# PRBonn/SHINE_mapping

Measured on NVIDIA H100. Metric: sdf_train_points_per_sec_fwd_bwd, higher is better.
Workload: dtype f32

## Files before the change

shine_mapping_b200/csrc/shine_b200.cu:

```cuda

#include <cuda_runtime.h>
#include <math.h>
#include <stdint.h>

#include <type_traits>

#include "shine_b200.h"

#ifndef SHINE_GATHER_GROUP
#define SHINE_GATHER_GROUP 2
#endif
#ifndef SHINE_TRAIN_MINB
#define SHINE_TRAIN_MINB 2
#endif
#ifndef SHINE_TRAIN_DECGRAD_MINB
#define SHINE_TRAIN_DECGRAD_MINB 1
#endif
#ifndef SHINE_INFER_MINB
#define SHINE_INFER_MINB 3
#endif

#include "shine_device.cuh"

namespace {


__global__ void hash_insert_kernel(HashSlot* __restrict__ slots, uint32_t mask, const int64_t* __restrict__ keys,
                                   const int32_t* __restrict__ corner_ids, int64_t n, int32_t node_base,
                                   int32_t* __restrict__ overflow) {
    const int64_t i = (int64_t)blockIdx.x * blockDim.x + threadIdx.x;
    if (i >= n) return;
// ... 214 lines not shown
}

__device__ __forceinline__ void to_afrag(const float (&v)[4], int odd, float (&a)[4]) {
    const float s0 = odd ? v[0] : v[2], s1 = odd ? v[1] : v[3];
    const float r0 = __shfl_xor_sync(kFull, s0, 1), r1 = __shfl_xor_sync(kFull, s1, 1);
    if (!odd) { a[0] = v[0]; a[2] = v[1]; a[1] = r0; a[3] = r1; }
    else      { a[0] = r0;   a[2] = r1;   a[1] = v[2]; a[3] = v[3]; }
}
__device__ __forceinline__ void from_cfrag(const float (&c)[4], int odd, float (&v)[4]) {
    const float s0 = odd ? c[0] : c[2], s1 = odd ? c[1] : c[3];
    const float r0 = __shfl_xor_sync(kFull, s0, 1), r1 = __shfl_xor_sync(kFull, s1, 1);
    if (!odd) { v[0] = c[0]; v[1] = c[1]; v[2] = r0; v[3] = r1; }
    else      { v[0] = r0;   v[1] = r1;   v[2] = c[2]; v[3] = c[3]; }
}

#define SHINE_ACC_DECL float dW2[2][4][4], dW1[2][4], db2p[4][2], db1p[4][2], dw3p[4][2]

__device__ __forceinline__ float reduce_scatter_g8(const float (&v)[8], int lane) {
    float a[4], b[2];
    const bool b4 = (lane & 16) != 0, b3 = (lane & 8) != 0, b2 = (lane & 4) != 0;
#pragma unroll
    for (int i = 0; i < 4; ++i) a[i] = (b4 ? v[4 + i] : v[i]) + __shfl_xor_sync(kFull, b4 ? v[i] : v[4 + i], 16);
#pragma unroll
    for (int i = 0; i < 2; ++i) b[i] = (b3 ? a[2 + i] : a[i]) + __shfl_xor_sync(kFull, b3 ? a[i] : a[2 + i], 8);
    return (b2 ? b[1] : b[0]) + __shfl_xor_sync(kFull, b2 ? b[0] : b[1], 4);
}

__device__ __forceinline__ int frag_chunk(int lane) { return lane ^ ((lane >> 2) & 6); }
template <int NTF>
__device__ __forceinline__ void load_afrag(const float* blk, int c, AFrag<NTF>& a) {
    const float4 v = *reinterpret_cast<const float4*>(blk + 4 * c);
    a.set_packed(v.x, v.y, v.z, v.w);
}
__device__ __forceinline__ void load_bfrag(const float* blk, int c, uint2& bh, uint2& bl) {
    const float2 v = *reinterpret_cast<const float2*>(blk + 2 * c);
    split_fast2(v.x, v.y, bh.x, bh.y, bl.x, bl.y);
}
__device__ __forceinline__ void stage_afrags(float* blk, const int (&sq)[2], const float (&c)[4][4]) {
#pragma unroll
    for (int mt = 0; mt < 2; ++mt)
#pragma unroll
        for (int q = 0; q < 2; ++q)
            *reinterpret_cast<float4*>(blk + 128 * mt + 4 * sq[q]) = make_float4(c[2 * mt][q], c[2 * mt + 1][q], c[2 * mt][2 + q], c[2 * mt + 1][2 + q]);
}
__device__ __forceinline__ int xfrag_word(int ks, int c) { return 64 * ks + 2 * (c ^ (8 * ks)); }
__device__ __forceinline__ void load_xfrag(const float* sx, int ks, int c, uint2& bh, uint2& bl) {
    const float2 v = *reinterpret_cast<const float2*>(sx + xfrag_word(ks, c));
    split_fast2(v.x, v.y, bh.x, bh.y, bl.x, bl.y);
}


constexpr int kGatherGroup = SHINE_GATHER_GROUP;

using shine_internal::StepParams;

struct SmemPlan {
    static constexpr int W1 = 0;
    static constexpr int W1T = W1 + 2 * kH * kF;
    static constexpr int W2 = W1T + 2 * kF * kWS;
    static constexpr int W3W2T = W2 + 2 * kH * kWS;
    static constexpr int B1 = W3W2T + 2 * kH * kWS;
    static constexpr int B2 = B1 + kH;
    static constexpr int W3 = B2 + kH;
    static constexpr int B3 = W3 + kH;
    static constexpr int GSCALE = B3 + 1;
    static constexpr int kDecGradFloats = kH * kF + kH + kH * kH + kH + kH + 1;
    static constexpr int ZSUM = B3 + 4;
    static constexpr int kZsumFloats = 8 * 5 * kTile;
    static constexpr int STAGE = ZSUM + kZsumFloats;
    static constexpr int SB2 = 0;
    static constexpr int SU = SB2;
    static constexpr int SA1 = SB2 + kTile * kH;
    static constexpr int SX = SA1 + kTile * kH;
    static constexpr int SA2 = SX + kTile * kF;
    static constexpr int SDP = SA2;
    static constexpr int kStagePerWarp = SA2 + kTile * kH;
    static constexpr int kStageGrouped = SDP + 2 * kTile;
    __host__ __device__ static constexpr int stage_per_warp(bool grouped) { return grouped ? kStageGrouped : kStagePerWarp; }
    static constexpr int kGroupPerLevel = 4 * kTile;
    static constexpr int kW2Part = kH * kH;
};

constexpr int kMaxGroupedRuns = 6;

__device__ __forceinline__ void red_add_f2(float* p, float a, float b) {
    asm volatile("red.global.add.v2.f32 [%0], {%1,%2};" ::"l"(p), "f"(a), "f"(b) : "memory");
}
__device__ __forceinline__ int group_slot(int p) { return 4 * (p & 3) + (p >> 2); }

template <int LMAX>
__device__ __forceinline__ void grouped_scatter(const StepParams& P, int L, int tile, const float* __restrict__ pt,
                                                float* __restrict__ dtile, const float (&dxc)[4], int lane) {
    const int g = lane >> 2, t = lane & 3;
    *reinterpret_cast<float2*>(dtile + g * kF + 2 * t) = make_float2(dxc[0], dxc[1]);
    *reinterpret_cast<float2*>(dtile + (g + 8) * kF + 2 * t) = make_float2(dxc[2], dxc[3]);
// ... 97 lines not shown
    shine_internal::BrickGrid g;
    __device__ __forceinline__ void load(const StepParams&, int64_t p, float& x, float& y, float& z) const {
        const int n1 = g.n + 1, per = n1 * n1 * n1;
        const int64_t b = p / per;
        const int r = (int)(p - b * per);
        const int i = r / (n1 * n1), j = (r / n1) % n1, k = r % n1;
        x = __fadd_rn(g.origin[0], __fmul_rn(g.spacing, (float)(__ldg(g.bricks + 3 * b) * g.n + i)));
        y = __fadd_rn(g.origin[1], __fmul_rn(g.spacing, (float)(__ldg(g.bricks + 3 * b + 1) * g.n + j)));
        z = __fadd_rn(g.origin[2], __fmul_rn(g.spacing, (float)(__ldg(g.bricks + 3 * b + 2) * g.n + k)));
    }
    __device__ __forceinline__ float out(float v) const { return -v; }
};

template <class Src>
constexpr int infer_min_blocks() { return std::is_same<Src, BatchCoords>::value ? SHINE_INFER_MINB : 2; }

template <int NTF, bool TRAIN, bool DEC_GRAD, int LMAX, bool GROUPED = false, class Src = BatchCoords>
__global__ void __launch_bounds__(256, !TRAIN ? infer_min_blocks<Src>() : (DEC_GRAD && !GROUPED) ? SHINE_TRAIN_DECGRAD_MINB : SHINE_TRAIN_MINB)
sdf_fused_kernel(const __grid_constant__ StepParams P, const __grid_constant__ Src src) {
    static_assert(std::is_same<Src, BatchCoords>::value || !TRAIN, "generated coordinates are for inference only");
    static_assert(!GROUPED || TRAIN, "the grouped scatter belongs to the training kernels");
    static_assert(!DEC_GRAD || TRAIN, "decoder gradients belong to the training kernels");
    static_assert(SmemPlan::kStagePerWarp >= SmemPlan::kDecGradFloats, "a warp's staging area holds its partial decoder gradient");
    static_assert(SmemPlan::kStageGrouped >= kH * kF + 3 * kH + 1, "a grouped warp's staging area holds its partial bias / dW1 gradients");
    static_assert(!(GROUPED && DEC_GRAD) ||
                      (SmemPlan::STAGE + 8 * (SmemPlan::kStageGrouped + LMAX * SmemPlan::kGroupPerLevel + SmemPlan::kW2Part)) * 4 + 1024 <=
                          227 * 1024 / SHINE_TRAIN_MINB,
                  "the grouped kernel's shared memory fits SHINE_TRAIN_MINB blocks/SM");
    extern __shared__ __align__(16) float smem[];
    uint32_t* smu = reinterpret_cast<uint32_t*>(smem);
    const int tid = threadIdx.x, lane = tid & 31, warp = tid >> 5;
    const int g = lane >> 2, t = lane & 3, odd = t & 1, half = t >> 1;
    constexpr int kWarps = 8;

    for (int i = tid; i < kH * kF; i += blockDim.x) {
        const int nrow = i / kF, k = i % kF;
        uint32_t hi, lo; split_tf32(P.dec.w1[i], hi, lo);
        smu[SmemPlan::W1 + i] = hi; smu[SmemPlan::W1 + kH * kF + i] = lo;
        smu[SmemPlan::W1T + k * kWS + nrow] = hi; smu[SmemPlan::W1T + kF * kWS + k * kWS + nrow] = lo;
    }
    for (int i = tid; i < kH * kH; i += blockDim.x) {
        const int nrow = i / kH, k = i % kH;
        const float w = P.dec.w2[i];
        uint32_t hi, lo; split_tf32(w, hi, lo);
        smu[SmemPlan::W2 + nrow * kWS + k] = hi; smu[SmemPlan::W2 + kH * kWS + nrow * kWS + k] = lo;
        split_tf32(__fmul_rn(P.dec.w3[nrow], w), hi, lo);
        smu[SmemPlan::W3W2T + k * kWS + nrow] = hi; smu[SmemPlan::W3W2T + kH * kWS + k * kWS + nrow] = lo;
    }
    if (tid < kH) {
        smem[SmemPlan::B1 + tid] = P.dec.b1 ? P.dec.b1[tid] : 0.f;
        smem[SmemPlan::B2 + tid] = P.dec.b2 ? P.dec.b2[tid] : 0.f;
        smem[SmemPlan::W3 + tid] = P.dec.w3[tid];
    }
    if (tid == 0) {
        smem[SmemPlan::B3] = P.dec.b3 ? P.dec.b3[0] : 0.f;
        smem[SmemPlan::GSCALE] = P.loss_scale * ((TRAIN && P.d_loss) ? __ldg(P.d_loss) : 1.0f);
    }
    constexpr int kPark = LMAX <= 4 ? 16 : 32;
    constexpr int kIdPark = 4 * LMAX;
    __syncthreads();
    SHINE_ACC_DECL;
#pragma unroll
    for (int a = 0; a < 2; ++a) {
#pragma unroll
        for (int b = 0; b < 4; ++b) { dW2[a][b][0] = dW2[a][b][1] = dW2[a][b][2] = dW2[a][b][3] = 0.f; }
        dW1[a][0] = dW1[a][1] = dW1[a][2] = dW1[a][3] = 0.f;
    }
#pragma unroll
    for (int j = 0; j < 4; ++j) { db2p[j][0] = db2p[j][1] = db1p[j][0] = db1p[j][1] = dw3p[j][0] = dw3p[j][1] = 0.f; }
    float dw3acc = 0.f, db2acc[4] = {0.f, 0.f, 0.f, 0.f}, db1acc[2][2] = {{0.f, 0.f}, {0.f, 0.f}};

    constexpr bool kSectorProbe = !TRAIN;
    const bool poly = P.oct.poly_interp != 0;
    const int L = P.oct.num_levels;

    float db3p = 0.f;
    float loss_acc = 0.f;

    constexpr int kStage = SmemPlan::stage_per_warp(GROUPED);
    float* stage = smem + SmemPlan::STAGE + warp * kStage;
    float* stX = stage + SmemPlan::SX;
    const int kp = g >> 2, fc = frag_chunk(lane);
    const int sq[2] = {frag_chunk(8 * t + (g & 3)), frag_chunk(8 * t + 4 + (g & 3))};
    float* gpt = smem + SmemPlan::STAGE + (DEC_GRAD ? 8 * kStage : 0) +
                 warp * (LMAX * SmemPlan::kGroupPerLevel + (DEC_GRAD ? 0 : kTile * kF));
    float* gdx = DEC_GRAD ? stX : gpt + LMAX * SmemPlan::kGroupPerLevel;
    float* w2p = smem + SmemPlan::STAGE + 8 * kStage + 8 * LMAX * SmemPlan::kGroupPerLevel + warp * SmemPlan::kW2Part;
    if (DEC_GRAD && GROUPED) {
#pragma unroll
        for (int f = 0; f < 8; ++f) *reinterpret_cast<float4*>(w2p + 128 * f + 4 * lane) = make_float4(0.f, 0.f, 0.f, 0.f);
    }

    const int warp_global = blockIdx.x * kWarps + warp;
    const int warp_stride = gridDim.x * kWarps;

    bool consecutive = true;
#pragma unroll
    for (int i = 1; i < LMAX; ++i)
        if (i < L && P.oct.lv[i].level != P.oct.lv[0].level - i) consecutive = false;

    float nx = 0.f, ny = 0.f, nz = 0.f, nlab = 0.f, nwgt = 1.f;
    bool nvalid = false;
    auto prefetch_inputs = [&](int tl) {
// ... 39 lines not shown
                phase = 2;
            } else {
                break;
            }
        }
        const bool virt = phase != 1;
        last_pass = phase == 2;
        advance = !virt;
        const int64_t base = (int64_t)tile * kTile;
        const int64_t myp = base + g + 8 * odd;
        const bool valid = virt ? false : nvalid;
        const float x = nx, y = ny, z = nz, lab = nlab, wgt = nwgt;
        if (!virt) prefetch_inputs(seq + warp_stride);

        float feat[4];
        float pk[kPark];
        float idp[kIdPark];
        uint32_t hitmask = 0;
        if constexpr (kSectorProbe) {
        {
            float acc[8] = {0.f, 0.f, 0.f, 0.f, 0.f, 0.f, 0.f, 0.f};
#pragma unroll
            for (int i = 0; i < kPark; ++i) pk[i] = 0.f;
            const unsigned long long key0 = valid ? morton_of(x, y, z, P.oct.lv[0].level) : 0ull;
#pragma unroll
            for (int g0 = 0; g0 < LMAX; g0 += kGatherGroup) {
                SlotSector sec[kGatherGroup];
#pragma unroll
                for (int j = 0; j < kGatherGroup; ++j) {
                    const int i = g0 + j;
                    if (i < L && valid) {
                        const shine_level& lv = P.oct.lv[i];
                        const unsigned long long kq = consecutive ? (key0 >> (3 * i)) : morton_of(x, y, z, lv.level);
                        sec[j] = ldg_sector(reinterpret_cast<const HashSlot*>(lv.hash_slots),
                                            hash_key(kq) & (lv.hash_capacity - 1), half);
                    }
                }
#pragma unroll
                for (int j = 0; j < kGatherGroup; ++j) {
                    const int i = g0 + j;
                    bool hit = false;
                    if (i < L && valid) {
                        const shine_level& lv = P.oct.lv[i];
                        const unsigned long long kq = consecutive ? (key0 >> (3 * i)) : morton_of(x, y, z, lv.level);
                        hit = resolve_sector(reinterpret_cast<const HashSlot*>(lv.hash_slots), lv.hash_capacity - 1, kq, half,
                                             sec[j]);
                    }
                    idp[4 * i] = __int_as_float(hit ? sec[j].ids[0] : -1); idp[4 * i + 1] = __int_as_float(hit ? sec[j].ids[1] : -1);
                    idp[4 * i + 2] = __int_as_float(hit ? sec[j].ids[2] : -1); idp[4 * i + 3] = __int_as_float(hit ? sec[j].ids[3] : -1);
                    if (hit) {
                        const shine_level& lv = P.oct.lv[i];
                        hitmask |= 1u << i;
                        float r0[8], r1[8], r2[8], r3[8];
                        ldg_row8(lv.features + (int64_t)sec[j].ids[0] * kF, r0);
                        ldg_row8(lv.features + (int64_t)sec[j].ids[1] * kF, r1);
                        ldg_row8(lv.features + (int64_t)sec[j].ids[2] * kF, r2);
                        ldg_row8(lv.features + (int64_t)sec[j].ids[3] * kF, r3);
                        Blend b; b.init(x, y, z, lv.level, poly);
                        pk[3 * i] = b.tx; pk[3 * i + 1] = b.ty; pk[3 * i + 2] = b.tz;
                        const float wz = half ? b.tz : b.uz;
                        const float w0 = __fmul_rn(__fmul_rn(b.ux, b.uy), wz), w1 = __fmul_rn(__fmul_rn(b.ux, b.ty), wz);
                        const float w2 = __fmul_rn(__fmul_rn(b.tx, b.uy), wz), w3 = __fmul_rn(__fmul_rn(b.tx, b.ty), wz);
                        blend4(acc, r0, r1, r2, r3, w0, w1, w2, w3);
                    }
                }
            }
#pragma unroll
            for (int q = 0; q < 4; ++q) {
                const float send = half ? acc[q] : acc[4 + q];
                const float recv = __shfl_xor_sync(kFull, send, 2);
                feat[q] = (half ? acc[4 + q] : acc[q]) + recv;
            }
        }
        } else {
        int slot[LMAX];
        {
            constexpr int LH = LMAX / 2;
            const unsigned long long key0 = valid ? morton_of(x, y, z, P.oct.lv[0].level) : 0ull;
            unsigned long long kq[LH];
            uint4 kf[LH];
            int mine[LH];
#pragma unroll
            for (int j = 0; j < LH; ++j) {
                const int i = 2 * j + half;
                mine[j] = -1;
                if (i < L && valid) {
                    const shine_level& lv = P.oct.lv[i];
                    const HashSlot* slots = reinterpret_cast<const HashSlot*>(lv.hash_slots);
                    kq[j] = consecutive ? (key0 >> (3 * i)) : morton_of(x, y, z, lv.level);
                    mine[j] = (int)(hash_key(kq[j]) & (lv.hash_capacity - 1));
                    kf[j] = __ldg(reinterpret_cast<const uint4*>(slots + mine[j]));
                }
            }
#pragma unroll
            for (int j = 0; j < LH; ++j) {
                const int i = 2 * j + half;
                if (i < L && valid) {
                    const unsigned long long k0 = ((unsigned long long)kf[j].y << 32) | kf[j].x;
                    if (k0 != kq[j]) {
                        if (k0 == kEmptyKey || (int)kf[j].w <= 0) {
                            mine[j] = -1;
                        } else {
                            const shine_level& lv = P.oct.lv[i];
                            mine[j] = probe_slot_from(reinterpret_cast<const HashSlot*>(lv.hash_slots),
                                                      lv.hash_capacity - 1, kq[j], (uint32_t)mine[j], (int)kf[j].w);
                        }
                    }
                }
            }
            __syncwarp();
#pragma unroll
            for (int j = 0; j < LH; ++j) {
                const int other = __shfl_xor_sync(kFull, mine[j], 2);
                slot[2 * j] = half ? other : mine[j];
                slot[2 * j + 1] = half ? mine[j] : other;
            }
        }

        {
            float acc[8] = {0.f, 0.f, 0.f, 0.f, 0.f, 0.f, 0.f, 0.f};
#pragma unroll
            for (int i = 0; i < kPark; ++i) pk[i] = 0.f;
#pragma unroll
            for (int i = 0; i < kIdPark; ++i) idp[i] = __int_as_float(-1);
#pragma unroll
            for (int i = 0; i < LMAX; ++i) {
                if (GROUPED && i < L && half) gpt[i * SmemPlan::kGroupPerLevel + 48 + group_slot(g + 8 * odd)] = __int_as_float(slot[i]);
                if (i < L && slot[i] >= 0) {
                    const shine_level& lv = P.oct.lv[i];
                    const HashSlot* slots = reinterpret_cast<const HashSlot*>(lv.hash_slots);
                    hitmask |= 1u << i;
                    const int4 id4 = ldg_i4(slot_ids(slots, slot[i], half));
                    idp[4 * i] = __int_as_float(id4.x); idp[4 * i + 1] = __int_as_float(id4.y);
                    idp[4 * i + 2] = __int_as_float(id4.z); idp[4 * i + 3] = __int_as_float(id4.w);
                    float r0[8], r1[8], r2[8], r3[8];
                    ldg_row8(lv.features + (int64_t)id4.x * kF, r0);
                    ldg_row8(lv.features + (int64_t)id4.y * kF, r1);
                    ldg_row8(lv.features + (int64_t)id4.z * kF, r2);
                    ldg_row8(lv.features + (int64_t)id4.w * kF, r3);
                    Blend b; b.init(x, y, z, lv.level, poly);
                    pk[3 * i] = b.tx; pk[3 * i + 1] = b.ty; pk[3 * i + 2] = b.tz;
                    if (GROUPED) {
                        float* lt = gpt + i * SmemPlan::kGroupPerLevel + group_slot(g + 8 * odd);
                        if (half) lt[32] = b.tz; else { lt[0] = b.tx; lt[16] = b.ty; }
                    }
                    const float wz = half ? b.tz : b.uz;
                    const float w0 = __fmul_rn(__fmul_rn(b.ux, b.uy), wz), w1 = __fmul_rn(__fmul_rn(b.ux, b.ty), wz);
                    const float w2 = __fmul_rn(__fmul_rn(b.tx, b.uy), wz), w3 = __fmul_rn(__fmul_rn(b.tx, b.ty), wz);
                    blend4(acc, r0, r1, r2, r3, w0, w1, w2, w3);
                }
            }
#pragma unroll
            for (int q = 0; q < 4; ++q) {
                const float send = half ? acc[q] : acc[4 + q];
                const float recv = __shfl_xor_sync(kFull, send, 2);
                feat[q] = (half ? acc[4 + q] : acc[q]) + recv;
// ... 34 lines not shown
            for (int j = 0; j < 4; ++j) {
                const float bA = smem[SmemPlan::B1 + 8 * j + 2 * t], bB = smem[SmemPlan::B1 + 8 * j + 2 * t + 1];
                h1[j][0] = bA; h1[j][1] = bB; h1[j][2] = bA; h1[j][3] = bB;
                const int off = (8 * j + g) * kF + 2 * t;
                bh[j] = *reinterpret_cast<const uint2*>(smu + SmemPlan::W1 + off);
                bl[j] = *reinterpret_cast<const uint2*>(smu + SmemPlan::W1 + kH * kF + off);
            }
            mma3x4<NTF>(h1, ax, bh, bl);
#pragma unroll
            for (int j = 0; j < 4; ++j) {
#pragma unroll
                for (int r = 0; r < 4; ++r) {
                    if (TRAIN && h1[j][r] > 0.f) m1 |= 1u << (4 * j + r);
                    h1[j][r] = fmaxf(h1[j][r], 0.f);
                }
                if (DEC_GRAD && !GROUPED) {
#pragma unroll
                    for (int q = 0; q < 2; ++q)
                        *reinterpret_cast<float2*>(stage + SmemPlan::SB2 + (4 * kp + j) * 64 + 2 * sq[q]) = make_float2(h1[j][q], h1[j][2 + q]);
                }
            }
            if (DEC_GRAD && GROUPED) stage_afrags(stage + SmemPlan::SU + 256 * kp, sq, h1);
        }
        float h2[4][4];
        {
#pragma unroll
            for (int j = 0; j < 4; ++j) {
                const float bA = smem[SmemPlan::B2 + 8 * j + 2 * t], bB = smem[SmemPlan::B2 + 8 * j + 2 * t + 1];
                h2[j][0] = bA; h2[j][1] = bB; h2[j][2] = bA; h2[j][3] = bB;
            }
#pragma unroll
            for (int kk = 0; kk < 4; ++kk) {
                AFrag<NTF> a; a.set(h1[kk][0], h1[kk][2], h1[kk][1], h1[kk][3]);
                uint2 bh[4], bl[4];
#pragma unroll
                for (int j = 0; j < 4; ++j) {
                    const int off = (8 * j + g) * kWS + 8 * kk + 2 * t;
// ... 26 lines not shown
        if (P.pred && half == 0 && valid) P.pred[myp] = src.out(pown);

        if (P.label == nullptr) continue;

        float dpo = 0.f;
        if (valid) {
            float li;
            bce_point(pown, lab, wgt, li, dpo);
            if (half == 0) loss_acc += wgt * li;
        }
        if (!TRAIN) continue;
        if (phase == 2) dpo = (g == 0 && odd == 0) ? zsum : 0.f;

        const float dpx = __shfl_xor_sync(kFull, dpo, 1);
        const float dp0 = odd ? dpx : dpo, dp8 = odd ? dpo : dpx;
        float db1t[4][2], dw3t[4][2];
        if (DEC_GRAD) {
#pragma unroll
            for (int j = 0; j < 4; ++j) { dw3t[j][0] = dp0 * h2[j][0] + dp8 * h2[j][2];  dw3t[j][1] = dp0 * h2[j][1] + dp8 * h2[j][3]; }
        }
        if (DEC_GRAD && !GROUPED) {
            float dh2[4][4];
#pragma unroll
            for (int j = 0; j < 4; ++j) {
                dh2[j][0] = h2[j][0] > 0.f ? dp0 * w3a[j] : 0.f; dh2[j][1] = h2[j][1] > 0.f ? dp0 * w3b[j] : 0.f;
                dh2[j][2] = h2[j][2] > 0.f ? dp8 * w3a[j] : 0.f; dh2[j][3] = h2[j][3] > 0.f ? dp8 * w3b[j] : 0.f;
                db2p[j][0] += dh2[j][0] + dh2[j][2]; db2p[j][1] += dh2[j][1] + dh2[j][3];
            }
            stage_afrags(stage + SmemPlan::SA2 + 256 * kp, sq, dh2);
        }
        if (DEC_GRAD && GROUPED) {
            uint32_t mg = 0, mg8 = 0;
#pragma unroll
            for (int j = 0; j < 4; ++j)
#pragma unroll
                for (int q = 0; q < 2; ++q) {
                    mg |= (h2[j][q] > 0.f ? 1u : 0u) << (8 * j + 2 * t + q);
                    mg8 |= (h2[j][2 + q] > 0.f ? 1u : 0u) << (8 * j + 2 * t + q);
                }
            mg |= __shfl_xor_sync(kFull, mg, 1); mg8 |= __shfl_xor_sync(kFull, mg8, 1);
            mg |= __shfl_xor_sync(kFull, mg, 2); mg8 |= __shfl_xor_sync(kFull, mg8, 2);
            if (t == 0) {
                *reinterpret_cast<float2*>(stage + SmemPlan::SDP + 2 * g) = make_float2(dp0, __uint_as_float(mg));
                *reinterpret_cast<float2*>(stage + SmemPlan::SDP + 2 * (g + 8)) = make_float2(dp8, __uint_as_float(mg8));
            }
        }
// ... 9 lines not shown
                                       h2[kk][1] > 0.f ? kTf32One : 0u, h2[kk][3] > 0.f ? kTf32One : 0u};
                uint2 bh[4], bl[4];
#pragma unroll
                for (int j = 0; j < 4; ++j) {
                    const int off = (8 * j + g) * kWS + 8 * kk + 2 * t;
                    bh[j] = *reinterpret_cast<const uint2*>(smu + SmemPlan::W3W2T + off);
                    bl[j] = *reinterpret_cast<const uint2*>(smu + SmemPlan::W3W2T + kH * kWS + off);
                }
                mma2x4_exact_a<NTF>(dh1, a, bh, bl);
            }
#pragma unroll
            for (int j = 0; j < 4; ++j) {
                dh1[j][0] *= dp0; dh1[j][1] *= dp0; dh1[j][2] *= dp8; dh1[j][3] *= dp8;
#pragma unroll
                for (int r = 0; r < 4; ++r) dh1[j][r] = ((m1 >> (4 * j + r)) & 1u) ? dh1[j][r] : 0.f;
                if (DEC_GRAD) { db1t[j][0] = dh1[j][0] + dh1[j][2]; db1t[j][1] = dh1[j][1] + dh1[j][3]; }
            }
            if (DEC_GRAD) stage_afrags(stage + SmemPlan::SA1 + 256 * kp, sq, dh1);
        }
        float dxc[4] = {0.f, 0.f, 0.f, 0.f};
        {
            float dxo[4] = {0.f, 0.f, 0.f, 0.f};
#pragma unroll
            for (int kk = 0; kk < 4; kk += 2) {
                AFrag<NTF> a0, a1;
                a0.set(dh1[kk][0], dh1[kk][2], dh1[kk][1], dh1[kk][3]);
                a1.set(dh1[kk + 1][0], dh1[kk + 1][2], dh1[kk + 1][1], dh1[kk + 1][3]);
                const int off = g * kWS + 8 * kk + 2 * t;
                const uint2 bh0 = *reinterpret_cast<const uint2*>(smu + SmemPlan::W1T + off);
                const uint2 bl0 = *reinterpret_cast<const uint2*>(smu + SmemPlan::W1T + kF * kWS + off);
                const uint2 bh1 = *reinterpret_cast<const uint2*>(smu + SmemPlan::W1T + off + 8);
                const uint2 bl1 = *reinterpret_cast<const uint2*>(smu + SmemPlan::W1T + kF * kWS + off + 8);
                mma3x2<NTF>(dxc, dxo, a0, a1, bh0, bl0, bh1, bl1);
            }
#pragma unroll
            for (int r = 0; r < 4; ++r) dxc[r] += dxo[r];
        }

        if (DEC_GRAD && !GROUPED) {
#pragma unroll
            for (int j = 0; j < 4; ++j) {
                db1p[j][0] += db1t[j][0]; db1p[j][1] += db1t[j][1];
                dw3p[j][0] += dw3t[j][0]; dw3p[j][1] += dw3t[j][1];
            }
            __syncwarp();
#pragma unroll
            for (int ks = 0; ks < 2; ++ks) {
                uint2 bh[4], bl[4];
#pragma unroll
                for (int nt = 0; nt < 4; ++nt) load_bfrag(stage + SmemPlan::SB2 + (4 * ks + nt) * 64, fc, bh[nt], bl[nt]);
#pragma unroll
                for (int mt = 0; mt < 2; ++mt) {
                    AFrag<NTF> a;
                    load_afrag(stage + SmemPlan::SA2 + (2 * ks + mt) * 128, fc, a);
                    mma3x4<NTF>(dW2[mt], a, bh, bl);
                }
            }
#pragma unroll
            for (int ks = 0; ks < 2; ++ks) {
                uint2 bh, bl;
                load_xfrag(stX, ks, fc, bh, bl);
                AFrag<NTF> a0, a1;
                load_afrag(stage + SmemPlan::SA1 + (2 * ks) * 128, fc, a0);
                load_afrag(stage + SmemPlan::SA1 + (2 * ks + 1) * 128, fc, a1);
                mma3x2<NTF>(dW1[0], dW1[1], a0, a1, bh, bl, bh, bl);
            }
            __syncwarp();
        }
        if (DEC_GRAD && GROUPED) {
            float cols[8];
#pragma unroll
            for (int j = 0; j < 4; ++j) { cols[2 * j] = dw3t[j][0]; cols[2 * j + 1] = dw3t[j][1]; }
            dw3acc += reduce_scatter_g8(cols, lane);
            __syncwarp();
            float dpk[2][2];
            uint32_t mk[2][2];
#pragma unroll
            for (int ks = 0; ks < 2; ++ks) {
                const float2 e0 = *reinterpret_cast<const float2*>(stage + SmemPlan::SDP + 2 * (4 * ks + t));
                const float2 e8 = *reinterpret_cast<const float2*>(stage + SmemPlan::SDP + 2 * (4 * ks + t + 8));
                dpk[ks][0] = e0.x; dpk[ks][1] = e8.x;
                mk[ks][0] = __float_as_uint(e0.y) >> g; mk[ks][1] = __float_as_uint(e8.y) >> g;
#pragma unroll
                for (int nt = 0; nt < 4; ++nt)
// ... 34 lines not shown
                    const float4 av = *reinterpret_cast<const float4*>(stage + SmemPlan::SA1 + (2 * ks + mt) * 128 + 4 * fc);
                    db1acc[mt][0] += av.x + av.z; db1acc[mt][1] += av.y + av.w;
                    a[mt].set_packed(av.x, av.y, av.z, av.w);
                }
                mma3x2<NTF>(dW1[0], dW1[1], a[0], a[1], bh, bl, bh, bl);
            }
            __syncwarp();
        }

        if constexpr (GROUPED) {
            grouped_scatter<LMAX>(P, L, tile, gpt, gdx, dxc, lane);
            continue;
        }
        float dx[4];
        from_cfrag(dxc, odd, dx);
        const float (&qk)[kPark] = pk;
        const float (&qid)[kIdPark] = idp;
#pragma unroll
        for (int i = 0; i < LMAX; ++i) {
            int ids[8];
#pragma unroll
            for (int k = 0; k < 4; ++k) {
                const int mine = __float_as_int(qid[4 * i + k]);
                const int other = __shfl_xor_sync(kFull, mine, 2);
                ids[2 * k] = half ? other : mine;
                ids[2 * k + 1] = half ? mine : other;
            }
            if (i < L && ids[0] >= 0) {
                const shine_level& lv = P.oct.lv[i];
                Blend b;
                b.tx = qk[3 * i]; b.ty = qk[3 * i + 1]; b.tz = qk[3 * i + 2];
                b.ux = __fsub_rn(1.0f, b.tx); b.uy = __fsub_rn(1.0f, b.ty); b.uz = __fsub_rn(1.0f, b.tz);
                float* gb = grad_base(lv, (uint32_t)tile, kF) + 4 * half;
                const float xy[4] = {__fmul_rn(b.ux, b.uy), __fmul_rn(b.ux, b.ty), __fmul_rn(b.tx, b.uy), __fmul_rn(b.tx, b.ty)};
                const f2_t zz = f2_pack(b.uz, b.tz), dx01 = f2_pack(dx[0], dx[1]), dx23 = f2_pack(dx[2], dx[3]);
#pragma unroll
                for (int c = 0; c < 8; c += 2) {
                    float w[2];
                    f2_unpack(f2_mul(f2_pack(xy[c >> 1], xy[c >> 1]), zz), w[0], w[1]);
#pragma unroll
                    for (int k = 0; k < 2; ++k) {
                        const f2_t wk = f2_pack(w[k], w[k]);
                        float g0, g1, g2, g3;
                        f2_unpack(f2_mul(wk, dx01), g0, g1); f2_unpack(f2_mul(wk, dx23), g2, g3);
                        red_add_f4(gb + (int64_t)ids[c + k] * kF, g0, g1, g2, g3);
                    }
                }
            }
        }
    }

    if (P.loss && P.label) {
#pragma unroll
        for (int o = 16; o > 0; o >>= 1) loss_acc += __shfl_xor_sync(kFull, loss_acc, o);
        if (lane == 0 && loss_acc != 0.f) atomicAdd(P.loss, loss_acc * P.loss_scale);
    }
    if (DEC_GRAD && GROUPED) {
        float* part = stage;
        constexpr int oB1 = 256, oB2 = 288, oW3 = 320, oB3 = 352, kVec = 353;
#pragma unroll
        for (int mt = 0; mt < 2; ++mt) {
            *reinterpret_cast<float2*>(part + (16 * mt + g) * kF + 2 * t) = make_float2(dW1[mt][0], dW1[mt][1]);
            *reinterpret_cast<float2*>(part + (16 * mt + g + 8) * kF + 2 * t) = make_float2(dW1[mt][2], dW1[mt][3]);
#pragma unroll
            for (int r = 0; r < 2; ++r) {
                float d1 = db1acc[mt][r], d2 = db2acc[2 * mt + r];
#pragma unroll
                for (int o = 1; o < 4; o <<= 1) { d1 += __shfl_xor_sync(kFull, d1, o); d2 += __shfl_xor_sync(kFull, d2, o); }
                if (t == 0) { part[oB1 + 16 * mt + g + 8 * r] = d1; part[oB2 + 8 * (2 * mt + r) + g] = d2; }
            }
        }
        part[oW3 + 8 * (g >> 1) + 2 * t + (g & 1)] = dw3acc;
// ... 9 lines not shown
                for (int w = 0; w < kWarps; ++w) v += smem[SmemPlan::STAGE + w * kStage + i];
                if (i < oB1) dst = P.dec.gw1 + i;
                else if (i < oB2) dst = P.dec.gb1 ? P.dec.gb1 + (i - oB1) : nullptr;
                else if (i < oW3) { v *= smem[SmemPlan::W3 + (i - oB2)]; dst = P.dec.gb2 ? P.dec.gb2 + (i - oB2) : nullptr; }
                else if (i < oB3) dst = P.dec.gw3 + (i - oW3);
                else dst = P.dec.gb3;
            } else {
                const int e = i - kVec, r = e / kH, c = e % kH;
                const int f = 128 * (4 * (c >> 4) + (r >> 3)) + 4 * (4 * (c & 7) + ((r & 7) >> 1)) + 2 * ((c >> 3) & 1) + (r & 1);
#pragma unroll
                for (int w = 0; w < kWarps; ++w) v += w2p[(w - warp) * SmemPlan::kW2Part + f];
                v *= smem[SmemPlan::W3 + r];
                dst = P.dec.gw2 + e;
            }
            if (v != 0.f && dst) atomicAdd(dst, v);
        }
    }
    if (DEC_GRAD && !GROUPED) {
        float* part = stage;
        constexpr int oW1 = 0, oB1 = 256, oW2 = 288, oB2 = 1312, oW3 = 1344, oB3 = 1376;
        __syncwarp();
#pragma unroll
        for (int mt = 0; mt < 2; ++mt) {
#pragma unroll
            for (int nt = 0; nt < 4; ++nt) {
                *reinterpret_cast<float2*>(part + oW2 + (16 * mt + g) * kH + 8 * nt + 2 * t) = make_float2(dW2[mt][nt][0], dW2[mt][nt][1]);
                *reinterpret_cast<float2*>(part + oW2 + (16 * mt + g + 8) * kH + 8 * nt + 2 * t) = make_float2(dW2[mt][nt][2], dW2[mt][nt][3]);
            }
            *reinterpret_cast<float2*>(part + oW1 + (16 * mt + g) * kF + 2 * t) = make_float2(dW1[mt][0], dW1[mt][1]);
            *reinterpret_cast<float2*>(part + oW1 + (16 * mt + g + 8) * kF + 2 * t) = make_float2(dW1[mt][2], dW1[mt][3]);
        }
#pragma unroll
        for (int j = 0; j < 4; ++j) {
#pragma unroll
            for (int q = 0; q < 2; ++q) {
                float a = db1p[j][q], b = db2p[j][q], c = dw3p[j][q];
#pragma unroll
                for (int o = 4; o < 32; o <<= 1) {
                    a += __shfl_xor_sync(kFull, a, o); b += __shfl_xor_sync(kFull, b, o); c += __shfl_xor_sync(kFull, c, o);
                }
                if (g == 0) {
                    part[oB1 + 8 * j + 2 * t + q] = a;
                    part[oB2 + 8 * j + 2 * t + q] = b;
                    part[oW3 + 8 * j + 2 * t + q] = c;
                }
            }
        }
#pragma unroll
        for (int o = 16; o > 0; o >>= 1) db3p += __shfl_xor_sync(kFull, db3p, o);
        if (lane == 0) part[oB3] = db3p;
        __syncthreads();
        for (int i = tid; i < SmemPlan::kDecGradFloats; i += blockDim.x) {
            float v = 0.f;
#pragma unroll
            for (int w = 0; w < kWarps; ++w) v += smem[SmemPlan::STAGE + w * kStage + i];
            if (v == 0.f) continue;
            float* dst;
            if (i < oB1) dst = P.dec.gw1 + i;
            else if (i < oW2) dst = P.dec.gb1 ? P.dec.gb1 + (i - oB1) : nullptr;
            else if (i < oB2) dst = P.dec.gw2 + (i - oW2);
            else if (i < oW3) dst = P.dec.gb2 ? P.dec.gb2 + (i - oB2) : nullptr;
            else if (i < oB3) dst = P.dec.gw3 + (i - oW3);
            else dst = P.dec.gb3;
            if (dst) atomicAdd(dst, v);
        }
    }
}


__global__ void __launch_bounds__(256) reduce_replicas_kernel(const __grid_constant__ shine_octree oct) {
    const shine_level& lv = oct.lv[blockIdx.y];
    if (lv.num_replicas <= 1 || !lv.grad_replicas || !lv.feature_grads) return;
    const int64_t n4 = (int64_t)lv.rows * oct.feature_dim / 4;
    float4* main4 = reinterpret_cast<float4*>(lv.feature_grads);
    float4* rep4 = reinterpret_cast<float4*>(lv.grad_replicas);
    const float4 zero = make_float4(0.f, 0.f, 0.f, 0.f);
    const int nrep = lv.num_replicas - 1;
    for (int64_t i = (int64_t)blockIdx.x * blockDim.x + threadIdx.x; i < n4; i += (int64_t)gridDim.x * blockDim.x) {
        float4 acc = main4[i];
// ... 73 lines not shown
        }
    }
}


int check_decoder(const shine_decoder* d, const shine_octree* o) {
    if (!d) return SHINE_ERR_INVALID_ARG;
    if (d->in_dim != kF || d->hidden != kH || d->mlp_level != 2 || o->feature_dim != kF) return SHINE_ERR_UNSUPPORTED;
    if (!d->w1 || !d->w2 || !d->w3) return SHINE_ERR_INVALID_ARG;
    return SHINE_OK;
}

template <int NTF, bool TRAIN, bool DEC_GRAD, int LMAX, bool GROUPED = false, class Src = BatchCoords>
int launch_fused_t(const StepParams& P, cudaStream_t st, const Src& src = Src()) {
    auto kern = sdf_fused_kernel<NTF, TRAIN, DEC_GRAD, LMAX, GROUPED, Src>;
    const int smem_floats = SmemPlan::STAGE + (DEC_GRAD ? 8 * SmemPlan::stage_per_warp(GROUPED) : 0) +
                            (GROUPED ? 8 * (LMAX * SmemPlan::kGroupPerLevel + (DEC_GRAD ? SmemPlan::kW2Part : kTile * kF)) : 0);
    const size_t smem_bytes = (size_t)smem_floats * sizeof(float);
    static int per_sm_by_dev[kMaxDevices] = {0};
    int& per_sm_cached = per_sm_by_dev[current_device()];
    cudaError_t e;
    if (per_sm_cached == 0) {
        e = cudaFuncSetAttribute(kern, cudaFuncAttributeMaxDynamicSharedMemorySize, (int)smem_bytes);
        if (e != cudaSuccess) return (int)e;
        e = cudaFuncSetAttribute(kern, cudaFuncAttributePreferredSharedMemoryCarveout, cudaSharedmemCarveoutMaxShared);
        if (e != cudaSuccess) return (int)e;
        int q = 1;
        e = cudaOccupancyMaxActiveBlocksPerMultiprocessor(&q, kern, 256, smem_bytes);
        if (e != cudaSuccess) return (int)e;
        cudaFuncAttributes fa;
        e = cudaFuncGetAttributes(&fa, kern);
        if (e != cudaSuccess) return (int)e;
        const int by_regs = fa.numRegs > 0 ? 65536 / (fa.numRegs * 256) : 1;
// ... 327 lines not shown
```

Before: 4.142 billion.

## Unify decoder-grad path and park corner ids in shared memory instead of registers

After: 4.161 billion (median of 6 runs). Within noise of the previous version (+0.5%).

```diff
diff --git a/shine_mapping_b200/csrc/shine_b200.cu b/shine_mapping_b200/csrc/shine_b200.cu
--- a/shine_mapping_b200/csrc/shine_b200.cu
+++ b/shine_mapping_b200/csrc/shine_b200.cu
@@ -12,9 +12,6 @@
 #endif
 #ifndef SHINE_TRAIN_MINB
 #define SHINE_TRAIN_MINB 2
-#endif
-#ifndef SHINE_TRAIN_DECGRAD_MINB
-#define SHINE_TRAIN_DECGRAD_MINB 1
 #endif
 #ifndef SHINE_INFER_MINB
 #define SHINE_INFER_MINB 3
@@ -259,8 +256,6 @@
     else      { v[0] = r0;   v[1] = r1;   v[2] = c[2]; v[3] = c[3]; }
 }
 
-#define SHINE_ACC_DECL float dW2[2][4][4], dW1[2][4], db2p[4][2], db1p[4][2], dw3p[4][2]
-
 __device__ __forceinline__ float reduce_scatter_g8(const float (&v)[8], int lane) {
     float a[4], b[2];
     const bool b4 = (lane & 16) != 0, b3 = (lane & 8) != 0, b2 = (lane & 4) != 0;
@@ -272,15 +267,6 @@
 }
 
 __device__ __forceinline__ int frag_chunk(int lane) { return lane ^ ((lane >> 2) & 6); }
-template <int NTF>
-__device__ __forceinline__ void load_afrag(const float* blk, int c, AFrag<NTF>& a) {
-    const float4 v = *reinterpret_cast<const float4*>(blk + 4 * c);
-    a.set_packed(v.x, v.y, v.z, v.w);
-}
-__device__ __forceinline__ void load_bfrag(const float* blk, int c, uint2& bh, uint2& bl) {
-    const float2 v = *reinterpret_cast<const float2*>(blk + 2 * c);
-    split_fast2(v.x, v.y, bh.x, bh.y, bl.x, bl.y);
-}
 __device__ __forceinline__ void stage_afrags(float* blk, const int (&sq)[2], const float (&c)[4][4]) {
 #pragma unroll
     for (int mt = 0; mt < 2; ++mt)
@@ -309,21 +295,21 @@
     static constexpr int W3 = B2 + kH;
     static constexpr int B3 = W3 + kH;
     static constexpr int GSCALE = B3 + 1;
-    static constexpr int kDecGradFloats = kH * kF + kH + kH * kH + kH + kH + 1;
     static constexpr int ZSUM = B3 + 4;
     static constexpr int kZsumFloats = 8 * 5 * kTile;
     static constexpr int STAGE = ZSUM + kZsumFloats;
-    static constexpr int SB2 = 0;
-    static constexpr int SU = SB2;
-    static constexpr int SA1 = SB2 + kTile * kH;
+    static constexpr int SU = 0;
+    static constexpr int SA1 = SU + kTile * kH;
     static constexpr int SX = SA1 + kTile * kH;
-    static constexpr int SA2 = SX + kTile * kF;
-    static constexpr int SDP = SA2;
-    static constexpr int kStagePerWarp = SA2 + kTile * kH;
-    static constexpr int kStageGrouped = SDP + 2 * kTile;
-    __host__ __device__ static constexpr int stage_per_warp(bool grouped) { return grouped ? kStageGrouped : kStagePerWarp; }
+    static constexpr int SDP = SX + kTile * kF;
+    static constexpr int kStagePerWarp = SDP + 2 * kTile;
     static constexpr int kGroupPerLevel = 4 * kTile;
     static constexpr int kW2Part = kH * kH;
+    static constexpr int kRowsPerLevel = 4 * 32;
+    __host__ __device__ static constexpr int floats(bool train, bool grouped, bool dec_grad, int lmax) {
+        return STAGE + (dec_grad ? 8 * (kStagePerWarp + kW2Part) : 0) +
+               (grouped ? 8 * (lmax * kGroupPerLevel + (dec_grad ? 0 : kTile * kF)) : train ? 8 * lmax * kRowsPerLevel : 0);
+    }
 };
 
 constexpr int kMaxGroupedRuns = 6;
@@ -451,19 +437,19 @@
 
 template <class Src>
 constexpr int infer_min_blocks() { return std::is_same<Src, BatchCoords>::value ? SHINE_INFER_MINB : 2; }
+template <int NTF, bool DEC_GRAD, int LMAX, bool GROUPED>
+__host__ __device__ constexpr int train_min_blocks() { return (DEC_GRAD && !GROUPED && LMAX > 4) ? 1 : SHINE_TRAIN_MINB; }
 
 template <int NTF, bool TRAIN, bool DEC_GRAD, int LMAX, bool GROUPED = false, class Src = BatchCoords>
-__global__ void __launch_bounds__(256, !TRAIN ? infer_min_blocks<Src>() : (DEC_GRAD && !GROUPED) ? SHINE_TRAIN_DECGRAD_MINB : SHINE_TRAIN_MINB)
+__global__ void __launch_bounds__(256, !TRAIN ? infer_min_blocks<Src>() : train_min_blocks<NTF, DEC_GRAD, LMAX, GROUPED>())
 sdf_fused_kernel(const __grid_constant__ StepParams P, const __grid_constant__ Src src) {
     static_assert(std::is_same<Src, BatchCoords>::value || !TRAIN, "generated coordinates are for inference only");
     static_assert(!GROUPED || TRAIN, "the grouped scatter belongs to the training kernels");
     static_assert(!DEC_GRAD || TRAIN, "decoder gradients belong to the training kernels");
-    static_assert(SmemPlan::kStagePerWarp >= SmemPlan::kDecGradFloats, "a warp's staging area holds its partial decoder gradient");
-    static_assert(SmemPlan::kStageGrouped >= kH * kF + 3 * kH + 1, "a grouped warp's staging area holds its partial bias / dW1 gradients");
-    static_assert(!(GROUPED && DEC_GRAD) ||
-                      (SmemPlan::STAGE + 8 * (SmemPlan::kStageGrouped + LMAX * SmemPlan::kGroupPerLevel + SmemPlan::kW2Part)) * 4 + 1024 <=
-                          227 * 1024 / SHINE_TRAIN_MINB,
-                  "the grouped kernel's shared memory fits SHINE_TRAIN_MINB blocks/SM");
+    static_assert(SmemPlan::kStagePerWarp >= kH * kF + 3 * kH + 1, "a warp's staging area holds its partial bias / dW1 gradients");
+    static_assert(!TRAIN || SmemPlan::floats(true, GROUPED, DEC_GRAD, LMAX) * 4 + 1024 <=
+                               227 * 1024 / train_min_blocks<NTF, DEC_GRAD, LMAX, GROUPED>(),
+                  "the training kernel's shared memory fits its minimum blocks/SM");
     extern __shared__ __align__(16) float smem[];
     uint32_t* smu = reinterpret_cast<uint32_t*>(smem);
     const int tid = threadIdx.x, lane = tid & 31, warp = tid >> 5;
@@ -493,18 +479,8 @@
         smem[SmemPlan::B3] = P.dec.b3 ? P.dec.b3[0] : 0.f;
         smem[SmemPlan::GSCALE] = P.loss_scale * ((TRAIN && P.d_loss) ? __ldg(P.d_loss) : 1.0f);
     }
-    constexpr int kPark = LMAX <= 4 ? 16 : 32;
-    constexpr int kIdPark = 4 * LMAX;
     __syncthreads();
-    SHINE_ACC_DECL;
-#pragma unroll
-    for (int a = 0; a < 2; ++a) {
-#pragma unroll
-        for (int b = 0; b < 4; ++b) { dW2[a][b][0] = dW2[a][b][1] = dW2[a][b][2] = dW2[a][b][3] = 0.f; }
-        dW1[a][0] = dW1[a][1] = dW1[a][2] = dW1[a][3] = 0.f;
-    }
-#pragma unroll
-    for (int j = 0; j < 4; ++j) { db2p[j][0] = db2p[j][1] = db1p[j][0] = db1p[j][1] = dw3p[j][0] = dw3p[j][1] = 0.f; }
+    float dW1[2][4] = {{0.f, 0.f, 0.f, 0.f}, {0.f, 0.f, 0.f, 0.f}};
     float dw3acc = 0.f, db2acc[4] = {0.f, 0.f, 0.f, 0.f}, db1acc[2][2] = {{0.f, 0.f}, {0.f, 0.f}};
 
     constexpr bool kSectorProbe = !TRAIN;
@@ -514,7 +490,7 @@
     float db3p = 0.f;
     float loss_acc = 0.f;
 
-    constexpr int kStage = SmemPlan::stage_per_warp(GROUPED);
+    constexpr int kStage = SmemPlan::kStagePerWarp;
     float* stage = smem + SmemPlan::STAGE + warp * kStage;
     float* stX = stage + SmemPlan::SX;
     const int kp = g >> 2, fc = frag_chunk(lane);
@@ -522,8 +498,11 @@
     float* gpt = smem + SmemPlan::STAGE + (DEC_GRAD ? 8 * kStage : 0) +
                  warp * (LMAX * SmemPlan::kGroupPerLevel + (DEC_GRAD ? 0 : kTile * kF));
     float* gdx = DEC_GRAD ? stX : gpt + LMAX * SmemPlan::kGroupPerLevel;
-    float* w2p = smem + SmemPlan::STAGE + 8 * kStage + 8 * LMAX * SmemPlan::kGroupPerLevel + warp * SmemPlan::kW2Part;
-    if (DEC_GRAD && GROUPED) {
+    float* w2p = smem + SmemPlan::STAGE + 8 * kStage + (GROUPED ? 8 * LMAX * SmemPlan::kGroupPerLevel : 0) +
+                 warp * SmemPlan::kW2Part;
+    int* rows = reinterpret_cast<int*>(smem + SmemPlan::STAGE + (DEC_GRAD ? 8 * (kStage + SmemPlan::kW2Part) : 0)) +
+                warp * LMAX * SmemPlan::kRowsPerLevel + 4 * lane;
+    if (DEC_GRAD) {
 #pragma unroll
         for (int f = 0; f < 8; ++f) *reinterpret_cast<float4*>(w2p + 128 * f + 4 * lane) = make_float4(0.f, 0.f, 0.f, 0.f);
     }
@@ -593,14 +572,10 @@
         if (!virt) prefetch_inputs(seq + warp_stride);
 
         float feat[4];
-        float pk[kPark];
-        float idp[kIdPark];
         uint32_t hitmask = 0;
         if constexpr (kSectorProbe) {
         {
             float acc[8] = {0.f, 0.f, 0.f, 0.f, 0.f, 0.f, 0.f, 0.f};
-#pragma unroll
-            for (int i = 0; i < kPark; ++i) pk[i] = 0.f;
             const unsigned long long key0 = valid ? morton_of(x, y, z, P.oct.lv[0].level) : 0ull;
 #pragma unroll
             for (int g0 = 0; g0 < LMAX; g0 += kGatherGroup) {
@@ -625,8 +600,6 @@
                         hit = resolve_sector(reinterpret_cast<const HashSlot*>(lv.hash_slots), lv.hash_capacity - 1, kq, half,
                                              sec[j]);
                     }
-                    idp[4 * i] = __int_as_float(hit ? sec[j].ids[0] : -1); idp[4 * i + 1] = __int_as_float(hit ? sec[j].ids[1] : -1);
-                    idp[4 * i + 2] = __int_as_float(hit ? sec[j].ids[2] : -1); idp[4 * i + 3] = __int_as_float(hit ? sec[j].ids[3] : -1);
                     if (hit) {
                         const shine_level& lv = P.oct.lv[i];
                         hitmask |= 1u << i;
@@ -636,7 +609,6 @@
                         ldg_row8(lv.features + (int64_t)sec[j].ids[2] * kF, r2);
                         ldg_row8(lv.features + (int64_t)sec[j].ids[3] * kF, r3);
                         Blend b; b.init(x, y, z, lv.level, poly);
-                        pk[3 * i] = b.tx; pk[3 * i + 1] = b.ty; pk[3 * i + 2] = b.tz;
                         const float wz = half ? b.tz : b.uz;
                         const float w0 = __fmul_rn(__fmul_rn(b.ux, b.uy), wz), w1 = __fmul_rn(__fmul_rn(b.ux, b.ty), wz);
                         const float w2 = __fmul_rn(__fmul_rn(b.tx, b.uy), wz), w3 = __fmul_rn(__fmul_rn(b.tx, b.ty), wz);
@@ -653,22 +625,26 @@
         }
         } else {
         int slot[LMAX];
+        int4 idv[LMAX];
         {
             constexpr int LH = LMAX / 2;
             const unsigned long long key0 = valid ? morton_of(x, y, z, P.oct.lv[0].level) : 0ull;
             unsigned long long kq[LH];
             uint4 kf[LH];
+            int4 ia[LH], ib[LH];
             int mine[LH];
 #pragma unroll
             for (int j = 0; j < LH; ++j) {
                 const int i = 2 * j + half;
                 mine[j] = -1;
+                ia[j] = ib[j] = make_int4(-1, -1, -1, -1);
                 if (i < L && valid) {
                     const shine_level& lv = P.oct.lv[i];
                     const HashSlot* slots = reinterpret_cast<const HashSlot*>(lv.hash_slots);
                     kq[j] = consecutive ? (key0 >> (3 * i)) : morton_of(x, y, z, lv.level);
                     mine[j] = (int)(hash_key(kq[j]) & (lv.hash_capacity - 1));
                     kf[j] = __ldg(reinterpret_cast<const uint4*>(slots + mine[j]));
+                    if (!GROUPED) { ia[j] = ldg_i4(slot_ids(slots, mine[j], 0)); ib[j] = ldg_i4(slot_ids(slots, mine[j], 1)); }
                 }
             }
 #pragma unroll
@@ -681,8 +657,9 @@
                             mine[j] = -1;
                         } else {
                             const shine_level& lv = P.oct.lv[i];
-                            mine[j] = probe_slot_from(reinterpret_cast<const HashSlot*>(lv.hash_slots),
-                                                      lv.hash_capacity - 1, kq[j], (uint32_t)mine[j], (int)kf[j].w);
+                            const HashSlot* slots = reinterpret_cast<const HashSlot*>(lv.hash_slots);
+                            mine[j] = probe_slot_from(slots, lv.hash_capacity - 1, kq[j], (uint32_t)mine[j], (int)kf[j].w);
+                            if (!GROUPED && mine[j] >= 0) { ia[j] = ldg_i4(slot_ids(slots, mine[j], 0)); ib[j] = ldg_i4(slot_ids(slots, mine[j], 1)); }
                         }
                     }
                 }
@@ -693,32 +670,33 @@
                 const int other = __shfl_xor_sync(kFull, mine[j], 2);
                 slot[2 * j] = half ? other : mine[j];
                 slot[2 * j + 1] = half ? mine[j] : other;
+                if (!GROUPED) {
+                    const int4 own = half ? ib[j] : ia[j], send = half ? ia[j] : ib[j];
+                    const int4 recv = make_int4(__shfl_xor_sync(kFull, send.x, 2), __shfl_xor_sync(kFull, send.y, 2),
+                                                __shfl_xor_sync(kFull, send.z, 2), __shfl_xor_sync(kFull, send.w, 2));
+                    idv[2 * j] = half ? recv : own;
+                    idv[2 * j + 1] = half ? own : recv;
+                }
             }
         }
 
         {
             float acc[8] = {0.f, 0.f, 0.f, 0.f, 0.f, 0.f, 0.f, 0.f};
 #pragma unroll
-            for (int i = 0; i < kPark; ++i) pk[i] = 0.f;
-#pragma unroll
-            for (int i = 0; i < kIdPark; ++i) idp[i] = __int_as_float(-1);
-#pragma unroll
             for (int i = 0; i < LMAX; ++i) {
                 if (GROUPED && i < L && half) gpt[i * SmemPlan::kGroupPerLevel + 48 + group_slot(g + 8 * odd)] = __int_as_float(slot[i]);
+                if (!GROUPED && i < L && slot[i] < 0) *reinterpret_cast<int4*>(rows + i * SmemPlan::kRowsPerLevel) = make_int4(-1, -1, -1, -1);
                 if (i < L && slot[i] >= 0) {
                     const shine_level& lv = P.oct.lv[i];
-                    const HashSlot* slots = reinterpret_cast<const HashSlot*>(lv.hash_slots);
                     hitmask |= 1u << i;
-                    const int4 id4 = ldg_i4(slot_ids(slots, slot[i], half));
-                    idp[4 * i] = __int_as_float(id4.x); idp[4 * i + 1] = __int_as_float(id4.y);
-                    idp[4 * i + 2] = __int_as_float(id4.z); idp[4 * i + 3] = __int_as_float(id4.w);
+                    const int4 id4 = GROUPED ? ldg_i4(slot_ids(reinterpret_cast<const HashSlot*>(lv.hash_slots), slot[i], half)) : idv[i];
+                    if (!GROUPED) *reinterpret_cast<int4*>(rows + i * SmemPlan::kRowsPerLevel) = id4;
                     float r0[8], r1[8], r2[8], r3[8];
                     ldg_row8(lv.features + (int64_t)id4.x * kF, r0);
                     ldg_row8(lv.features + (int64_t)id4.y * kF, r1);
                     ldg_row8(lv.features + (int64_t)id4.z * kF, r2);
                     ldg_row8(lv.features + (int64_t)id4.w * kF, r3);
                     Blend b; b.init(x, y, z, lv.level, poly);
-                    pk[3 * i] = b.tx; pk[3 * i + 1] = b.ty; pk[3 * i + 2] = b.tz;
                     if (GROUPED) {
                         float* lt = gpt + i * SmemPlan::kGroupPerLevel + group_slot(g + 8 * odd);
                         if (half) lt[32] = b.tz; else { lt[0] = b.tx; lt[16] = b.ty; }
@@ -783,13 +761,8 @@
                     if (TRAIN && h1[j][r] > 0.f) m1 |= 1u << (4 * j + r);
                     h1[j][r] = fmaxf(h1[j][r], 0.f);
                 }
-                if (DEC_GRAD && !GROUPED) {
-#pragma unroll
-                    for (int q = 0; q < 2; ++q)
-                        *reinterpret_cast<float2*>(stage + SmemPlan::SB2 + (4 * kp + j) * 64 + 2 * sq[q]) = make_float2(h1[j][q], h1[j][2 + q]);
-                }
-            }
-            if (DEC_GRAD && GROUPED) stage_afrags(stage + SmemPlan::SU + 256 * kp, sq, h1);
+            }
+            if (DEC_GRAD) stage_afrags(stage + SmemPlan::SU + 256 * kp, sq, h1);
         }
         float h2[4][4];
         {
@@ -846,22 +819,10 @@
 
         const float dpx = __shfl_xor_sync(kFull, dpo, 1);
         const float dp0 = odd ? dpx : dpo, dp8 = odd ? dpo : dpx;
-        float db1t[4][2], dw3t[4][2];
+        float dw3t[4][2];
         if (DEC_GRAD) {
 #pragma unroll
             for (int j = 0; j < 4; ++j) { dw3t[j][0] = dp0 * h2[j][0] + dp8 * h2[j][2];  dw3t[j][1] = dp0 * h2[j][1] + dp8 * h2[j][3]; }
-        }
-        if (DEC_GRAD && !GROUPED) {
-            float dh2[4][4];
-#pragma unroll
-            for (int j = 0; j < 4; ++j) {
-                dh2[j][0] = h2[j][0] > 0.f ? dp0 * w3a[j] : 0.f; dh2[j][1] = h2[j][1] > 0.f ? dp0 * w3b[j] : 0.f;
-                dh2[j][2] = h2[j][2] > 0.f ? dp8 * w3a[j] : 0.f; dh2[j][3] = h2[j][3] > 0.f ? dp8 * w3b[j] : 0.f;
-                db2p[j][0] += dh2[j][0] + dh2[j][2]; db2p[j][1] += dh2[j][1] + dh2[j][3];
-            }
-            stage_afrags(stage + SmemPlan::SA2 + 256 * kp, sq, dh2);
-        }
-        if (DEC_GRAD && GROUPED) {
             uint32_t mg = 0, mg8 = 0;
 #pragma unroll
             for (int j = 0; j < 4; ++j)
@@ -901,7 +862,6 @@
                 dh1[j][0] *= dp0; dh1[j][1] *= dp0; dh1[j][2] *= dp8; dh1[j][3] *= dp8;
 #pragma unroll
                 for (int r = 0; r < 4; ++r) dh1[j][r] = ((m1 >> (4 * j + r)) & 1u) ? dh1[j][r] : 0.f;
-                if (DEC_GRAD) { db1t[j][0] = dh1[j][0] + dh1[j][2]; db1t[j][1] = dh1[j][1] + dh1[j][3]; }
             }
             if (DEC_GRAD) stage_afrags(stage + SmemPlan::SA1 + 256 * kp, sq, dh1);
         }
@@ -924,37 +884,7 @@
             for (int r = 0; r < 4; ++r) dxc[r] += dxo[r];
         }
 
-        if (DEC_GRAD && !GROUPED) {
-#pragma unroll
-            for (int j = 0; j < 4; ++j) {
-                db1p[j][0] += db1t[j][0]; db1p[j][1] += db1t[j][1];
-                dw3p[j][0] += dw3t[j][0]; dw3p[j][1] += dw3t[j][1];
-            }
-            __syncwarp();
-#pragma unroll
-            for (int ks = 0; ks < 2; ++ks) {
-                uint2 bh[4], bl[4];
-#pragma unroll
-                for (int nt = 0; nt < 4; ++nt) load_bfrag(stage + SmemPlan::SB2 + (4 * ks + nt) * 64, fc, bh[nt], bl[nt]);
-#pragma unroll
-                for (int mt = 0; mt < 2; ++mt) {
-                    AFrag<NTF> a;
-                    load_afrag(stage + SmemPlan::SA2 + (2 * ks + mt) * 128, fc, a);
-                    mma3x4<NTF>(dW2[mt], a, bh, bl);
-                }
-            }
-#pragma unroll
-            for (int ks = 0; ks < 2; ++ks) {
-                uint2 bh, bl;
-                load_xfrag(stX, ks, fc, bh, bl);
-                AFrag<NTF> a0, a1;
-                load_afrag(stage + SmemPlan::SA1 + (2 * ks) * 128, fc, a0);
-                load_afrag(stage + SmemPlan::SA1 + (2 * ks + 1) * 128, fc, a1);
-                mma3x2<NTF>(dW1[0], dW1[1], a0, a1, bh, bl, bh, bl);
-            }
-            __syncwarp();
-        }
-        if (DEC_GRAD && GROUPED) {
+        if (DEC_GRAD) {
             float cols[8];
 #pragma unroll
             for (int j = 0; j < 4; ++j) { cols[2 * j] = dw3t[j][0]; cols[2 * j + 1] = dw3t[j][1]; }
@@ -1019,23 +949,21 @@
         }
         float dx[4];
         from_cfrag(dxc, odd, dx);
-        const float (&qk)[kPark] = pk;
-        const float (&qid)[kIdPark] = idp;
 #pragma unroll
         for (int i = 0; i < LMAX; ++i) {
+            if (i >= L) break;
+            const int4 own = *reinterpret_cast<const int4*>(rows + i * SmemPlan::kRowsPerLevel);
+            const int mine[4] = {own.x, own.y, own.z, own.w};
             int ids[8];
 #pragma unroll
             for (int k = 0; k < 4; ++k) {
-                const int mine = __float_as_int(qid[4 * i + k]);
-                const int other = __shfl_xor_sync(kFull, mine, 2);
-                ids[2 * k] = half ? other : mine;
-                ids[2 * k + 1] = half ? mine : other;
-            }
-            if (i < L && ids[0] >= 0) {
+                const int other = __shfl_xor_sync(kFull, mine[k], 2);
+                ids[2 * k] = half ? other : mine[k];
+                ids[2 * k + 1] = half ? mine[k] : other;
+            }
+            if (ids[0] >= 0) {
                 const shine_level& lv = P.oct.lv[i];
-                Blend b;
-                b.tx = qk[3 * i]; b.ty = qk[3 * i + 1]; b.tz = qk[3 * i + 2];
-                b.ux = __fsub_rn(1.0f, b.tx); b.uy = __fsub_rn(1.0f, b.ty); b.uz = __fsub_rn(1.0f, b.tz);
+                Blend b; b.init(x, y, z, lv.level, poly);
                 float* gb = grad_base(lv, (uint32_t)tile, kF) + 4 * half;
                 const float xy[4] = {__fmul_rn(b.ux, b.uy), __fmul_rn(b.ux, b.ty), __fmul_rn(b.tx, b.uy), __fmul_rn(b.tx, b.ty)};
                 const f2_t zz = f2_pack(b.uz, b.tz), dx01 = f2_pack(dx[0], dx[1]), dx23 = f2_pack(dx[2], dx[3]);
@@ -1060,7 +988,7 @@
         for (int o = 16; o > 0; o >>= 1) loss_acc += __shfl_xor_sync(kFull, loss_acc, o);
         if (lane == 0 && loss_acc != 0.f) atomicAdd(P.loss, loss_acc * P.loss_scale);
     }
-    if (DEC_GRAD && GROUPED) {
+    if (DEC_GRAD) {
         float* part = stage;
         constexpr int oB1 = 256, oB2 = 288, oW3 = 320, oB3 = 352, kVec = 353;
 #pragma unroll
@@ -1100,55 +1028,6 @@
                 dst = P.dec.gw2 + e;
             }
             if (v != 0.f && dst) atomicAdd(dst, v);
-        }
-    }
-    if (DEC_GRAD && !GROUPED) {
-        float* part = stage;
-        constexpr int oW1 = 0, oB1 = 256, oW2 = 288, oB2 = 1312, oW3 = 1344, oB3 = 1376;
-        __syncwarp();
-#pragma unroll
-        for (int mt = 0; mt < 2; ++mt) {
-#pragma unroll
-            for (int nt = 0; nt < 4; ++nt) {
-                *reinterpret_cast<float2*>(part + oW2 + (16 * mt + g) * kH + 8 * nt + 2 * t) = make_float2(dW2[mt][nt][0], dW2[mt][nt][1]);
-                *reinterpret_cast<float2*>(part + oW2 + (16 * mt + g + 8) * kH + 8 * nt + 2 * t) = make_float2(dW2[mt][nt][2], dW2[mt][nt][3]);
-            }
-            *reinterpret_cast<float2*>(part + oW1 + (16 * mt + g) * kF + 2 * t) = make_float2(dW1[mt][0], dW1[mt][1]);
-            *reinterpret_cast<float2*>(part + oW1 + (16 * mt + g + 8) * kF + 2 * t) = make_float2(dW1[mt][2], dW1[mt][3]);
-        }
-#pragma unroll
-        for (int j = 0; j < 4; ++j) {
-#pragma unroll
-            for (int q = 0; q < 2; ++q) {
-                float a = db1p[j][q], b = db2p[j][q], c = dw3p[j][q];
-#pragma unroll
-                for (int o = 4; o < 32; o <<= 1) {
-                    a += __shfl_xor_sync(kFull, a, o); b += __shfl_xor_sync(kFull, b, o); c += __shfl_xor_sync(kFull, c, o);
-                }
-                if (g == 0) {
-                    part[oB1 + 8 * j + 2 * t + q] = a;
-                    part[oB2 + 8 * j + 2 * t + q] = b;
-                    part[oW3 + 8 * j + 2 * t + q] = c;
-                }
-            }
-        }
-#pragma unroll
-        for (int o = 16; o > 0; o >>= 1) db3p += __shfl_xor_sync(kFull, db3p, o);
-        if (lane == 0) part[oB3] = db3p;
-        __syncthreads();
-        for (int i = tid; i < SmemPlan::kDecGradFloats; i += blockDim.x) {
-            float v = 0.f;
-#pragma unroll
-            for (int w = 0; w < kWarps; ++w) v += smem[SmemPlan::STAGE + w * kStage + i];
-            if (v == 0.f) continue;
-            float* dst;
-            if (i < oB1) dst = P.dec.gw1 + i;
-            else if (i < oW2) dst = P.dec.gb1 ? P.dec.gb1 + (i - oB1) : nullptr;
-            else if (i < oB2) dst = P.dec.gw2 + (i - oW2);
-            else if (i < oW3) dst = P.dec.gb2 ? P.dec.gb2 + (i - oB2) : nullptr;
-            else if (i < oB3) dst = P.dec.gw3 + (i - oW3);
-            else dst = P.dec.gb3;
-            if (dst) atomicAdd(dst, v);
         }
     }
 }
@@ -1252,9 +1131,7 @@
 template <int NTF, bool TRAIN, bool DEC_GRAD, int LMAX, bool GROUPED = false, class Src = BatchCoords>
 int launch_fused_t(const StepParams& P, cudaStream_t st, const Src& src = Src()) {
     auto kern = sdf_fused_kernel<NTF, TRAIN, DEC_GRAD, LMAX, GROUPED, Src>;
-    const int smem_floats = SmemPlan::STAGE + (DEC_GRAD ? 8 * SmemPlan::stage_per_warp(GROUPED) : 0) +
-                            (GROUPED ? 8 * (LMAX * SmemPlan::kGroupPerLevel + (DEC_GRAD ? SmemPlan::kW2Part : kTile * kF)) : 0);
-    const size_t smem_bytes = (size_t)smem_floats * sizeof(float);
+    const size_t smem_bytes = (size_t)SmemPlan::floats(TRAIN, GROUPED, DEC_GRAD, LMAX) * sizeof(float);
     static int per_sm_by_dev[kMaxDevices] = {0};
     int& per_sm_cached = per_sm_by_dev[current_device()];
     cudaError_t e;
```
